# romi/plant-3d-vision

Hardware: AMD Instinct MI355X
Metric: Mvoxels*views/sec space-carve, 512^3 x 72 views per MI355X (higher is better)
Workload: dtype f32

## Files before the change

### include/spacecarve_tuning.h

```cpp
#ifndef SPACECARVE_TUNING_H
#define SPACECARVE_TUNING_H

#define SC_OPT_COMPACT 5

#define SC_OPT_DENSE_VIEWS 6
#define SC_OPT_STAGE1_VIEWS 7
#define SC_OPT_LIST_BLOCKS 8
#define SC_OPT_VIEW_GROUP 9
#define SC_OPT_BRICK 10
#define SC_OPT_STAGE2_VIEWS 12
#define SC_OPT_PACK_ROWS 13
#define SC_OPT_DEFER_STORES 14
#define SC_OPT_DEFER_SHARE 15
#define SC_OPT_FULL_BRICKS 19
#define SC_OPT_AVG_BRICK 20
#define SC_OPT_AVG_TILE_F32 29
#define SC_OPT_STAGE1_STORE_SHARE 17
#define SC_OPT_STAGE1_LIST_BLOCKS 21
#define SC_OPT_PACK_RIDE 22
#define SC_OPT_BRICK_WALKERS 23
#define SC_OPT_FILL_BLOCKS 25
#define SC_OPT_FINAL_VOXELS 24
#define SC_OPT_VIEW_BRICK 26
#define SC_OPT_STAGE1_VOXELS 30
#define SC_OPT_FLAG_VIEWS 11
#define SC_OPT_BULK_MIN 32
#define SC_OPT_ITEM_BIAS 33
#define SC_OPT_UNIT_BLOCKS 34
#define SC_OPT_BULK_FLOOR 35
#define SC_OPT_BULK_ADAPT SC_OPT_BULK_FLOOR

#define SC_OPT_LIST_CAP 38
#define SC_OPT_HOST_PACK 39
#define SC_OPT_HOST_THREADS 40
#define SC_OPT_LDS_TILES 41
#define SC_OPT_BULK_LIVE 42
#define SC_OPT_SAFE_KERNELS 43
#define SC_OPT_DENSE_EXTRA 44
#define SC_OPT_SPEC_SHARE 45
#define SC_OPT_SPEC_BLOCKS 46
#define SC_OPT_LATE_ROAD 47
#define SC_OPT_UNIT_CULL 37

#endif
```

### plant-3d-vision_amd/_native.py

```python
import ctypes
import importlib.util
import os
import subprocess
import sys
import threading

import numpy as np

_PKG_DIR = os.path.dirname(os.path.abspath(__file__))
LIB_PATH = os.path.join(_PKG_DIR, "libspacecarve.so")
_ALT_LIB = os.environ.get("SPACECARVE_LIB", "")
if _ALT_LIB:
    LIB_PATH = os.path.abspath(_ALT_LIB)
HEADER_PATH = os.path.join(os.path.dirname(_PKG_DIR), "include", "spacecarve.h")

SC_OK = 0
SC_ERR_INVALID, SC_ERR_DEVICE, SC_ERR_NOMEM, SC_ERR_STATE = -1, -2, -3, -4
SC_MODE_CARVE, SC_MODE_AVERAGE = 0, 1
SC_CREATE_DEFERRED = 1
SC_MASK_U8, SC_MASK_I32, SC_MASK_F32, SC_MASK_U8_INV, SC_MASK_BOOL_INV = 0, 1, 2, 3, 4
SC_MASK_U8_LUT = 5
SC_OPT_VIEWS_PER_LAUNCH, SC_OPT_VIEW_ORDER, SC_OPT_TIME_KERNELS, SC_OPT_MAX_PENDING = 1, 2, 3, 4
SC_OPT_COMPACT, SC_OPT_DENSE_VIEWS, SC_OPT_STAGE1_VIEWS, SC_OPT_LIST_BLOCKS = 5, 6, 7, 8
SC_OPT_VIEW_GROUP, SC_OPT_BRICK, SC_OPT_FLAG_VIEWS, SC_OPT_STAGE2_VIEWS = 9, 10, 11, 12
SC_KERNEL_CARVE, SC_KERNEL_AVERAGE, SC_KERNEL_PACK, SC_KERNEL_FILL, SC_KERNEL_LIST = 0, 1, 2, 3, 4
SC_KERNEL_FLAGS, SC_KERNEL_STEP = 5, 6
SC_OPT_PACK_ROWS, SC_OPT_DEFER_STORES, SC_OPT_DEFER_SHARE = 13, 14, 15
SC_OPT_FULL_BRICKS, SC_OPT_AVG_BRICK = 19, 20
SC_OPT_STAGE1_STORE_SHARE, SC_OPT_STAGE1_LIST_BLOCKS = 17, 21
SC_OPT_PACK_RIDE, SC_OPT_BRICK_WALKERS, SC_OPT_FILL_BLOCKS, SC_OPT_FINAL_VOXELS = 22, 23, 25, 24
SC_OPT_VIEW_BRICK, SC_OPT_AVG_TILE_F32, SC_OPT_STAGE1_VOXELS, SC_OPT_RESERVE_EVENTS = 26, 29, 30, 31
SC_OPT_BULK_MIN, SC_OPT_ITEM_BIAS, SC_OPT_UNIT_BLOCKS, SC_OPT_BULK_FLOOR = 32, 33, 34, 35
SC_OPT_BULK_ADAPT = SC_OPT_BULK_FLOOR
SC_OPT_UNIT_CULL, SC_OPT_LIST_CAP, SC_OPT_HOST_PACK, SC_OPT_HOST_THREADS, SC_OPT_LDS_TILES, SC_OPT_BULK_LIVE, SC_OPT_SAFE_KERNELS = 37, 38, 39, 40, 41, 42, 43
SC_OPT_DENSE_EXTRA = 44
SC_OPT_SPEC_SHARE, SC_OPT_SPEC_BLOCKS, SC_OPT_LATE_ROAD = 45, 46, 47
SC_FILTER_LINEAR, SC_FILTER_EXCESS_GREEN = 0, 1
SC_FOOT = {"t0": 0, "t90": 1, "t180": 2, "t270": 3, "diamond": 4, "square": 5}

_SIGNATURES = {
    "sc_abi_version": ("i", []),
    "sc_last_error": ("s", []),
    "sc_device_count": ("i", ["p"]),
    "sc_create": ("i", ["p", "q", "q", "q", "p", "f", "i", "f", "i"]),
    "sc_create_slab": ("i", ["p", "q", "q", "q", "q", "q", "p", "f", "i", "f", "i"]),
    "sc_create_cyclic": ("i", ["p", "q", "q", "q", "q", "q", "p", "f", "i", "f", "i"]),
    "sc_prewarm": ("i", ["i"]),
    "sc_prewarm_wait": ("v", []),
    "sc_create_ex": ("i", ["p", "q", "q", "q", "q", "q", "q", "p", "f", "i", "f", "i", "i"]),
    "sc_setup_times": ("i", ["p", "p"]),
    "sc_destroy": ("v", ["p"]),
    "sc_clear": ("i", ["p"]),
    "sc_set_option": ("i", ["p", "i", "q"]),
    "sc_set_stream": ("i", ["p", "p"]),
    "sc_order_after": ("i", ["p", "p"]),
    "sc_order_before": ("i", ["p", "p"]),
    "sc_set_lut": ("i", ["p", "p"]),
    "sc_process_view": ("i", ["p", "p", "p", "p", "p", "i", "i", "i", "q"]),
    "sc_process_views": ("i", ["p", "i", "p", "p", "p", "p", "i", "i", "i", "q"]),
    "sc_process_views_device": ("i", ["p", "i", "p", "p", "p", "p", "i", "i", "i"]),
    "sc_process_png_views": ("i", ["p", "i", "p", "p", "p", "p", "p", "i", "i"]),
    "sc_average_labels": ("i", ["p", "i", "i", "p", "p", "p", "p", "i", "i"]),
    "sc_average_labels_fused_count": ("q", []),
    "sc_flush": ("i", ["p"]),
    "sc_synchronize": ("i", ["p"]),
    "sc_get_values": ("i", ["p", "p"]),
    "sc_get_values_i8": ("i", ["p", "p"]),
    "sc_values_device_ptr": ("i", ["p", "p"]),
    "sc_num_voxels": ("q", ["p"]),
# ... 988 lines not shown
```

### plant-3d-vision_amd/csrc/sc_bricks.h

```cpp

template <bool ALL_SAFE = false>
__device__ __forceinline__ void two_views(const ViewDesc &da, const ViewDesc &db, bool two, float x, float y,
                                          const float (&z)[4], unsigned long long (&alive)[4], unsigned long long (&kept)[4]) {
    const float aax = da.R[0] * x + da.R[1] * y, aay = da.R[3] * x + da.R[4] * y, aaz = da.R[6] * x + da.R[7] * y;
    const float bax = db.R[0] * x + db.R[1] * y, bay = db.R[3] * x + db.R[4] * y, baz = db.R[6] * x + db.R[7] * y;
    const uint32_t rowa = (uint32_t)da.strip, rowb = (uint32_t)db.strip;
    unsigned long long oka[4], okb[4];
    uint32_t wa[4], wb[4];
    int sha[4], shb[4];
#pragma unroll
    for (int e = 0; e < 4; ++e) {
        int v;
        bool ok = project<ALL_SAFE>(aax, aay, aaz, z[e], da, sha[e], v, oka[e]);
        wa[e] = load_mask_at(da.mask, ok ? mask_byte_offset(sha[e], v, rowa) : 0u);
        ok = project<ALL_SAFE>(bax, bay, baz, z[e], db, shb[e], v, okb[e]);
        wb[e] = load_mask_at(db.mask, ok ? mask_byte_offset(shb[e], v, rowb) : 0u);
    }
    const unsigned long long second = two ? ~0ull : 0ull;
#pragma unroll
    for (int e = 0; e < 4; ++e) {
        unsigned long long fg = __ballot(__builtin_amdgcn_ubfe(wa[e], (uint32_t)sha[e], 1u) != 0u);
        unsigned long long seen = oka[e] & alive[e];
        alive[e] &= ~(seen & ~fg);
        kept[e] |= seen & fg;
// ... 138 lines not shown
        unsigned long long body = culled & ~last;
        while (body != 0) {
            const uint32_t bz = (uint32_t)__builtin_ctzll(body);
            body &= body - 1;
            asm volatile("global_store_dwordx4 %0, %1, %2 nt" ::"v"(voff), "v"(minus), "s"(wbase + bz * 256u) : "memory");
        }
        if ((culled & last) != 0 && tail_ok)
            asm volatile("global_store_dwordx4 %0, %1, %2 nt" ::"v"(voff), "v"(minus), "s"(wbase + (bricks_z - 1u) * 256u) : "memory");
        asm volatile("s_nop 1" ::"v"(minus));
    }
    unsigned long long rest = full | untouched;
    if (rest == 0) return;
    int32_t *col = labels + ((uint64_t)il * g.ny + j) * g.nzp;
    while (rest != 0) {
        const uint32_t bz = (uint32_t)__builtin_ctzll(rest);
        rest &= rest - 1;
        const bool isfull = (full >> bz) & 1ull;
        const uint32_t k0 = bz * kBrickZ + l16 * 4;
        if (k0 >= g.nz) continue;
        if (!isfull || fill.fresh) {
            const int32_t val = isfull ? fill.kept : fill.init;
            const v4i vv = {val, val, val, val};
            __builtin_nontemporal_store(vv, reinterpret_cast<v4i *>(col + k0));
        } else {
            const uint32_t n = min(4u, g.nz - k0);
            for (uint32_t e = 0; e < n; ++e)
                if (col[k0 + e] == 0) col[k0 + e] = 1;
        }
    }
}

#ifdef SC_TRACE_DENSE
__device__ uint32_t g_dense_trace[8192 * 8];
#endif
constexpr int kConfirmWaves = 8;
struct UnitRoad {
    int32_t *labels;
    int32_t init, fresh;
    uint32_t nbricks;
};

__global__ __launch_bounds__(64 * kConfirmWaves) void brick_confirm_kernel(
    GridDesc g, const ViewDesc *__restrict__ views, int v0, int v1, uint32_t bricks_y, uint32_t bricks_z,
    uint8_t *__restrict__ flags, const uint32_t *__restrict__ cands, uint32_t cand_per, uint32_t *__restrict__ late,
    ListCtl *ctl, uint32_t parity, UnitRoad ur) {
    if (v0 >= v1) return;
    uint32_t ncand[kCandSub], gfirst[kCandSub + 1];
    gfirst[0] = 0;
#pragma unroll
    for (int s = 0; s < kCandSub; ++s) {
        ncand[s] = ctl->ncand[parity][s].n;
        gfirst[s + 1] = gfirst[s] + ((ncand[s] + 63u) >> 6);
    }
    __shared__ unsigned long long s_full[kConfirmWaves], s_seen[kConfirmWaves];
    __shared__ unsigned long long s_road, s_rseen;
    const uint32_t wave = __builtin_amdgcn_readfirstlane(threadIdx.x >> 6), lane = threadIdx.x & 63u;
    const uint32_t per_plane = bricks_y * bricks_z;
    for (uint32_t grp = blockIdx.x; grp < gfirst[kCandSub]; grp += gridDim.x) {
        uint32_t sub = 0, first = 0, n = ncand[0];
#pragma unroll
        for (int s = 1; s < kCandSub; ++s)
            if (grp >= gfirst[s]) { sub = (uint32_t)s; first = gfirst[s]; n = ncand[s]; }
        const uint32_t idx = (grp - first) * 64u + lane;
        const bool isc = idx < n;
        const uint32_t lb = isc ? cands[(size_t)sub * cand_per * 64u + idx] : 0u;
        const uint32_t fl = isc ? flags[lb] : 0u;
// ... 43 lines not shown
                const uint32_t src = (uint32_t)__builtin_ctzll(mm);
                const uint32_t b = __builtin_amdgcn_readlane(lb, src);
                const bool seen = (ms >> src) & 1ull;
                const uint32_t bil = b / per_plane, brem = b - bil * per_plane;
                const uint32_t bby = brem / bricks_z, bbz = brem - bby * bricks_z;
                const uint32_t k0 = bbz * kBrickZ + (lane & 15u) * 4u;
#pragma unroll
                for (uint32_t i = 0; i < 4u; ++i) {
                    const uint32_t j = bby * kBrickY + i * 4u + (lane >> 4);
                    if (j >= g.ny || k0 >= g.nz) continue;
                    int32_t *p = ur.labels + ((uint64_t)bil * g.ny + j) * g.nzp + k0;
                    if (ur.fresh) {
                        const int32_t val = (seen && ur.init == 0) ? 1 : ur.init;
                        *reinterpret_cast<int4 *>(p) = make_int4(val, val, val, val);
                    } else if (seen) {
                        int4 q = *reinterpret_cast<const int4 *>(p);
                        const bool changed = q.x == 0 || q.y == 0 || q.z == 0 || q.w == 0;
                        q.x = q.x == 0 ? 1 : q.x; q.y = q.y == 0 ? 1 : q.y; q.z = q.z == 0 ? 1 : q.z; q.w = q.w == 0 ? 1 : q.w;
                        if (changed) *reinterpret_cast<int4 *>(p) = q;
                    }
                }
            }
        }
        __syncthreads();
    }
}

template <bool FRESH, bool ALL_SAFE = false>
__global__ __launch_bounds__(kBlock) __attribute__((amdgpu_num_sgpr(102))) void carve_brick_kernel(int32_t *__restrict__ labels, GridDesc g,
                                                             const ViewDesc *__restrict__ views,
                                                             int nviews, int32_t init, Append ap,
                                                             uint32_t bricks_y, uint32_t bricks_z,
                                                             const uint8_t *__restrict__ flags,
                                                             const uint32_t *__restrict__ live,
                                                             ListCtl *ctl, uint32_t nwalkers,
                                                             PackJob ride, int pack_rows,
                                                             uint32_t parity, int nverd_arg, uint32_t verd_max_live,
                                                             uint32_t bulk_min_live, int nextra) {
    if (blockIdx.x >= nwalkers) {
        const uint32_t b = blockIdx.x - nwalkers;
        if (pack_rows == 0) pack_band_block(ride, b);
        else if (pack_rows == 1) pack16_block<1>(ride, b);
        else if (pack_rows == 2) pack16_block<2>(ride, b);
        else if (pack_rows == 8) pack16_block<8>(ride, b);
        else pack16_block<4>(ride, b);
        return;
    }
    const uint32_t nlive = ctl->nlive[parity];
    const int nverd = nlive <= verd_max_live ? nverd_arg : 0;
    if (nlive < bulk_min_live) ap.bulk = nullptr;
    const uint32_t lane = threadIdx.x & 63;
    const uint32_t per_plane = bricks_y * bricks_z;
    const uint32_t xcd = blockIdx.x & 7u;
    const uint32_t per_xcd = (nwalkers >> 3) * (kBlock / 64);
    bool first = true;
    uint32_t misses = 0, turn = 0;
#ifdef SC_TRACE_DENSE
    const uint64_t tr0 = wall_clock64();
    uint32_t tr_bricks = 0, tr_units = 0, tr_verd = 0, tr_unit = 0, tr_tick = 0;
#endif
    for (;;) {
#ifdef SC_TRACE_DENSE
        const uint64_t tra = wall_clock64();
#endif
        uint32_t t = (blockIdx.x >> 3) * (kBlock / 64) + (threadIdx.x >> 6);
        if (!first) {
            const uint32_t nc = min(8u, per_xcd);
            const uint32_t c = t % nc;
            uint32_t n = 0;
            if (lane == 0) n = atomicAdd(&ctl->xcd_next[xcd * 8u + c].n, 1u);
            n = __builtin_amdgcn_readfirstlane(n);
            t = per_xcd + ((n / kXcdRun) * nc + c) * kXcdRun + (n % kXcdRun);
        }
        first = false;
        t = __builtin_amdgcn_readfirstlane(t);
        const uint32_t entry = ((t / kXcdRun) * 8u + xcd) * kXcdRun + (t % kXcdRun);
        if ((t / kXcdRun) * 8u * kXcdRun >= nlive) break;
        if (entry >= nlive) continue;
        const uint32_t lb = __builtin_amdgcn_readfirstlane(live[entry]);
        const uint32_t il = lb / per_plane;
        const uint32_t rem = lb - il * per_plane;
        const uint32_t by = rem / bricks_z, bz = rem - by * bricks_z;
        uint32_t culled = 0;
#ifdef SC_TRACE_DENSE
        const uint64_t trb = wall_clock64();
        tr_tick += (uint32_t)(trb - tra);
        ++tr_bricks;
#endif
        const bool ask = nverd > 0 && (misses < 8u || (turn & 7u) == 0u);
        ++turn;
        if (ask) {
            const uint32_t u = lane >> 4, vq = lane & 15u;
            uint32_t v = 0u;
            if ((int)vq < nverd) {
                const ViewDesc d = views[vq];
                const float x = g.ox + (float)(int)(il * g.istride + g.i0) * g.vs;
                v = rect_verdict_cells(d, g, x, (int)(by * kBrickY), (int)(by * kBrickY) + kBrickY - 1,
                                       (int)(bz * kBrickZ + u * 16u), (int)(bz * kBrickZ + u * 16u) + 15);
            }
            const unsigned long long e = __ballot(v == 1u);
            culled = ((e & 0xffffull) ? 1u : 0u) | (((e >> 16) & 0xffffull) ? 2u : 0u) |
                     (((e >> 32) & 0xffffull) ? 4u : 0u) | ((e >> 48) ? 8u : 0u);
            misses = culled ? 0u : misses + 1u;
        }
#ifdef SC_TRACE_DENSE
        const uint64_t trc = wall_clock64();
        tr_verd += (uint32_t)(trc - trb);
#endif
        const uint32_t j = by * kBrickY + (lane >> 2);
        for (uint32_t u = 0; u < 4u; ++u) {
            const uint32_t k0 = bz * kBrickZ + u * 16u + (lane & 3u) * 4u;
            if ((culled >> u) & 1u) {
                if (j < g.ny && k0 < g.nz)
                    *reinterpret_cast<int4 *>(labels + ((uint64_t)il * g.ny + j) * g.nzp + k0) = make_int4(-1, -1, -1, -1);
                continue;
            }
            brick_voxels<FRESH, ALL_SAFE>(labels, g, views, nviews, init, ap, il, j, k0, lb, lane, u, nextra);
#ifdef SC_TRACE_DENSE
            ++tr_units;
#endif
        }
#ifdef SC_TRACE_DENSE
        tr_unit += (uint32_t)(wall_clock64() - trc);
#endif
    }
#ifdef SC_TRACE_DENSE
    if (lane == 0) {
        const uint32_t w = blockIdx.x * 4u + (threadIdx.x >> 6);
        if (w < 8192u) {
            uint32_t *o = g_dense_trace + w * 8u;
            o[0] = (uint32_t)tr0; o[1] = (uint32_t)wall_clock64(); o[2] = tr_bricks; o[3] = tr_units;
            o[4] = tr_verd; o[5] = tr_unit; o[6] = tr_tick; o[7] = 0;
        }
    }
#endif
}

template <bool FRESH>
__global__ __launch_bounds__(kBlock) __attribute__((amdgpu_num_sgpr(102))) void carve_brick_light_kernel(
    int32_t *__restrict__ labels, GridDesc g, const ViewDesc *__restrict__ views, int nviews, int32_t init,
    uint32_t bricks_y, uint32_t bricks_z, const uint32_t *__restrict__ live, const uint32_t *__restrict__ fill_list,
    const ListCtl *ctl, uint32_t nwalkers, uint32_t parity) {
    const uint32_t wave = __builtin_amdgcn_readfirstlane(threadIdx.x >> 6), lane = threadIdx.x & 63;
    const uint32_t per_plane = bricks_y * bricks_z;
    if (blockIdx.x >= nwalkers) {
        const uint32_t nfill = ctl->nfill[parity], nfillers = gridDim.x - nwalkers;
        const bool vec = (g.nzp & 3u) == 0;
        const int32_t kept = init == 0 ? 1 : init;
        for (uint32_t base = (blockIdx.x - nwalkers) * 64u; base < nfill; base += nfillers * 64u) {
            const uint32_t mine = (base + lane < nfill) ? fill_list[base + lane] : 0u;
            const uint32_t n = min(64u, nfill - base);
            for (uint32_t q = 0; q < n; ++q) {
                const uint32_t ent = __builtin_amdgcn_readlane(mine, q);
                const bool isfull = (ent >> 31) != 0, isunt = ((ent >> 30) & 1u) != 0;
                if (isunt && !FRESH) continue;
                const uint32_t lb = ent & 0x3fffffffu;
                const uint32_t il = lb / per_plane;
                const uint32_t rem = lb - il * per_plane;
                const uint32_t by = rem / bricks_z, bz = rem - by * bricks_z;
                const uint32_t j = by * kBrickY + wave * 4 + (lane >> 4), k0 = bz * kBrickZ + (lane & 15) * 4;
                if (j >= g.ny || k0 >= g.nz) continue;
                int32_t *p = labels + ((uint64_t)il * g.ny + j) * g.nzp + k0;
                const uint32_t nv4 = min(4u, g.nz - k0);
                if (!isfull || FRESH) {
                    const int32_t val = isunt ? init : (isfull ? kept : -1);
                    if (vec) {
                        typedef int v4i __attribute__((ext_vector_type(4)));
                        v4i vv = {val, val, val, val};
                        __builtin_nontemporal_store(vv, reinterpret_cast<v4i *>(p));
                    } else {
                        for (uint32_t e = 0; e < nv4; ++e) p[e] = val;
                    }
                } else {
                    for (uint32_t e = 0; e < nv4; ++e)
                        if (p[e] == 0) p[e] = 1;
                }
            }
        }
        return;
    }
    const uint32_t nlive = ctl->nlive[parity];
    const Append none{nullptr, nullptr, 0u, 0u, nullptr, 0u, 0u};
    const uint32_t xcd = blockIdx.x & 7u, seq = blockIdx.x >> 3, per_xcd = nwalkers >> 3;
    for (uint32_t t = seq; ; t += per_xcd) {
        const uint32_t entry = ((t / kXcdRun) * 8u + xcd) * kXcdRun + (t % kXcdRun);
        if ((t / kXcdRun) * 8u * kXcdRun >= nlive) break;
        if (entry >= nlive) continue;
        const uint32_t lb = live[entry];
        const uint32_t il = lb / per_plane;
        const uint32_t rem = lb - il * per_plane;
        const uint32_t by = rem / bricks_z, bz = rem - by * bricks_z;
        const uint32_t j = by * kBrickY + wave * 4 + (lane >> 4);
        brick_voxels<FRESH>(labels, g, views, nviews, init, none, il, j, bz * kBrickZ + (lane & 15) * 4, lb, lane);
    }
}

template <bool FRESH, bool VEC>
__global__ __launch_bounds__(kBlock) void carve_kernel_1(int32_t *__restrict__ labels, GridDesc g,
                                                         ViewDesc view, int32_t init) {
    static_assert(VEC, "rows are whole 16-byte groups: the state is always read and written as int4");
    constexpr int G = !FRESH ? kStreamGroups : 1;
    uint32_t lb = spread_block(blockIdx.x, gridDim.x);
    uint64_t grp = (uint64_t)lb * (kBlock * G) + threadIdx.x;
    Append none{nullptr, nullptr, 0u, 0u, nullptr, 0u, 0u};
    int4 cur = make_int4(-1, -1, -1, -1);
    typedef int v4i __attribute__((ext_vector_type(4)));
    auto stream_load = [&](uint64_t gidx) {
        v4i q = __builtin_nontemporal_load(reinterpret_cast<const v4i *>(labels + gidx * 4));
        return make_int4(q.x, q.y, q.z, q.w);
    };
    if (!FRESH && grp < g.ngroups) cur = stream_load(grp);
#pragma unroll 1
    for (int s = 0; s < G; ++s, grp += kBlock) {
        int4 nxt = make_int4(-1, -1, -1, -1);
        if (G > 1 && s + 1 < G && grp + kBlock < g.ngroups)
            nxt = stream_load(grp + kBlock);
        if (grp < g.ngroups) carve_group<FRESH>(labels, g, &view, 1, init, grp, cur, none);
        cur = nxt;
    }
}
```

### plant-3d-vision_amd/csrc/sc_engine.h

```cpp

struct sc_engine {
    int device = 0;
    int mode = SC_MODE_CARVE;
    int64_t nx = 0, ny = 0, nz = 0, i0 = 0, istride = 1, planes = 0, n = 0;
    int64_t nzp = 0;
    int64_t npitch = 0;
    void *dense = nullptr;
    float origin[3] = {0, 0, 0};
    float vs = 1.0f;
    float default_value = 0.0f;
    void *state = nullptr;
    bool fresh = true;

    hipStream_t own_stream = nullptr, stream = nullptr;
    std::thread setup_thread;
    bool setup_pending = false;
    int setup_rc = SC_OK;
    std::string setup_err;
    double setup_ms = 0.0;
    double setup_waited_ms = 0.0;

    std::vector<ViewDesc> pending;
    ViewDesc *views_dev = nullptr;
    ViewDesc *views_pin = nullptr;
// ... 32 lines not shown
    bool sparse_late = false;
    hipEvent_t sparse_busy[2] = {nullptr, nullptr}, packed_busy = nullptr;
    bool sparse_busy_armed[2] = {false, false}, packed_busy_armed = false;
    size_t packed_cap = 0;
    SparseHeader *sparse_hdr_pin[2] = {nullptr, nullptr};
    size_t wire_stage_words = 0;
    int64_t unit_cull = 1;
    uint32_t *late = nullptr;
    uint32_t *bulk = nullptr;
    uint32_t bulkcap = 0;
    int64_t bulk_min = 128;
    bool last_bulk = false;
    uint4 *items = nullptr;
    uint32_t itemcap = 0;
    int64_t bulk_floor = 8192;
    int64_t bulk_live = 2;
    int64_t list_cap = 0, list_cap_built = 0;
    uint32_t *fill_list = nullptr;
    uint64_t flag_launches = 0;
    uint32_t last_parity = 0;
    struct DeferredBatch {
        bool on = false;
        const void *raw = nullptr;
        int V = 0, H = 0, W = 0, dtype = 0;
        int64_t row_stride = 0, view_stride = 0;
    } deferred;
    int64_t flag_views = 8;
    float *lut_dev = nullptr;

    uint32_t *lists = nullptr;
    ListCtl *ctl = nullptr;
    uint32_t subcap = 0;

    int64_t late_road = 1;
    int64_t safe_kernels = 1;
    int64_t host_pack = 1;
    struct HostBits {
        char *pin = nullptr, *dev = nullptr;
        size_t cap = 0, used = 0;
        hipEvent_t ev = nullptr;
        bool armed = false;
    } hb[2];
    int hb_cur = 0;
    std::vector<BitsRec> hp_pending;

    void *pin[kSlots] = {nullptr, nullptr, nullptr, nullptr};
    void *raw[kSlots] = {nullptr, nullptr, nullptr, nullptr};
    hipEvent_t slot_ev[kSlots] = {nullptr, nullptr, nullptr, nullptr};
    bool slot_armed[kSlots] = {false, false, false, false};
    size_t slot_bytes = 0;
    int next_slot = 0;

    int64_t views_per_launch = 0;
    int64_t view_order = 1;
    int64_t time_kernels = 0;
    int64_t max_pending = 256;
    int64_t compact = 1;
    int64_t brick = 1;
    int64_t dense_views = 2;
    int64_t stage1_views = 6;

    std::vector<TimedLaunch> timed[kNumKernels];
    hipEvent_t step_start = nullptr;
    bool step_open = false;
    hipEvent_t span_start = nullptr;
    bool span_open = false;
// ... 711 lines not shown
```

### plant-3d-vision_amd/csrc/sc_sparse.h

```cpp

constexpr uint32_t kSparseMagic = 0x50534353u;
constexpr uint32_t kSparseBrickBytes = kBrickY * kBrickZ / 4;
constexpr uint32_t kSparseMixed = 2u;

struct SparseHeader {
    uint32_t magic, version, bits, nbricks;
    uint32_t cap, nmixed, planes, ny;
    uint32_t nz, bricks_y, bricks_z, first;
    uint32_t stride;
    uint32_t nread;
    uint32_t pad[2];
};
static_assert(sizeof(SparseHeader) == 64, "SparseHeader layout");

struct SparseLayout {
    uint64_t codes, ids, payload, total;
};
__host__ __device__ inline SparseLayout sparse_layout(uint32_t nbricks, uint32_t cap) {
    SparseLayout l;
    l.codes = 64;
    l.ids = l.codes + (((uint64_t)nbricks + 63u) & ~(uint64_t)63u);
    l.payload = l.ids + (((uint64_t)cap * 4u + 63u) & ~(uint64_t)63u);
    l.total = l.payload + (uint64_t)cap * kSparseBrickBytes;
    return l;
}

struct SparseCounters {
    uint32_t nmixed, pad0[31];
    uint32_t nwork, pad1[31];
    uint32_t done, pad2[31];
};

struct SparseScan {
    const uint8_t *flags;
    uint32_t nbricks;
    int32_t level;
    uint32_t code_full, code_untouched;
    uint32_t *work;
};
struct SparseLists {
    const uint32_t *list0, *list1, *list2;
    const uint32_t *count0, *count1, *count2;
    int32_t step0, step1, step2;
};

constexpr uint32_t kSparseTurn = 8;

__global__ __launch_bounds__(kBlock) void sparse_pack_kernel(const int32_t *__restrict__ labels, GridDesc g, uint32_t bricks_y,
                                                            uint32_t bricks_z, SparseScan sc, uint32_t nscan, SparseLists sl,
                                                            char *__restrict__ wire, SparseHeader hdr, SparseCounters *cnt,
                                                            SparseCounters *cnt_next) {
    const SparseLayout lay = sparse_layout(hdr.nbricks, hdr.cap);
    uint8_t *codes = reinterpret_cast<uint8_t *>(wire + lay.codes);
    const uint32_t lane = threadIdx.x & 63u;
    const unsigned long long below = (lane == 0) ? 0ull : (~0ull >> (64 - lane));
    if (blockIdx.x < nscan) {
        const uint32_t b = blockIdx.x * kBlock + threadIdx.x;
        bool unknown = false;
        if (b < sc.nbricks) {
            uint32_t code = kSparseMixed;
            if (sc.level == 2) {
                const uint32_t f = sc.flags[b];
                code = (f == 1u || f == 4u) ? 3u : (f == 2u ? sc.code_full : (f == 6u ? sc.code_untouched : kSparseMixed));
            } else if (sc.level == 1) {
                code = sc.flags[b] != 0 ? 3u : kSparseMixed;
            }
            unknown = code == kSparseMixed;
            if (!unknown) codes[b] = (uint8_t)code;
        }
        if (sc.work != nullptr) {
            const unsigned long long m = __ballot(unknown);
            if (m != 0) {
                uint32_t base = 0;
                if (lane == 0) base = atomicAdd(&cnt->nwork, (uint32_t)__popcll(m));
                base = __shfl(base, 0);
                if (unknown) sc.work[base + (uint32_t)__popcll(m & below)] = b;
            }
        }
        return;
    }
    if (blockIdx.x == nscan && threadIdx.x == 0 && cnt_next != nullptr) {
        cnt_next->nmixed = 0u;
        cnt_next->nwork = 0u;
        cnt_next->done = 0u;
    }
    uint32_t *ids = reinterpret_cast<uint32_t *>(wire + lay.ids);
    uint32_t *payload = reinterpret_cast<uint32_t *>(wire + lay.payload);
    __shared__ uint32_t s_mixed[kBlock / 64], s_base;
    const uint32_t wave = __builtin_amdgcn_readfirstlane(threadIdx.x >> 6);
    const uint32_t npack = gridDim.x - nscan;
    uint32_t n0 = 0, n1 = 0, n2 = 0;
    if (sl.list0 != nullptr) n0 = *sl.count0;
    if (sl.list1 != nullptr) n1 = *sl.count1;
    if (sl.list2 != nullptr) n2 = *sl.count2;
    n0 = min(n0, hdr.nbricks); n1 = min(n1, hdr.nbricks); n2 = min(n2, hdr.nbricks);
    const uint32_t total = n0 + n1 + n2;
    const uint32_t per_plane = bricks_y * bricks_z;
    const uint32_t jl = lane >> 2, kq = (lane & 3u) * 16u;
    constexpr uint32_t kBlockTurn = kSparseTurn * (kBlock / 64);
    for (uint32_t tb = (blockIdx.x - nscan) * kBlockTurn; tb < total; tb += npack * kBlockTurn) {
        uint32_t mine = 0xffffffffu, j0 = 0, kb = 0, off_lo = 0, off_hi = 0;
        {
            const uint32_t t = tb + wave * kSparseTurn + lane;
            if (lane < kSparseTurn && t < total) {
                const uint32_t *lp = t < n0 ? sl.list0 : (t < n0 + n1 ? sl.list1 : sl.list2);
                const int64_t at = t < n0 ? (int64_t)t * sl.step0
                                          : (t < n0 + n1 ? (int64_t)(t - n0) * sl.step1 : (int64_t)(t - n0 - n1) * sl.step2);
                mine = lp[at];
                if (mine >= hdr.nbricks) mine = 0xffffffffu;
            }
            if (mine != 0xffffffffu) {
                const uint32_t il = mine / per_plane, rem = mine - il * per_plane;
                const uint32_t by = rem / bricks_z, bz = rem - by * bricks_z;
                j0 = by * kBrickY;
                kb = bz * kBrickZ;
                const uint64_t off = ((uint64_t)il * g.ny + j0) * g.nzp + kb;
                off_lo = (uint32_t)off;
                off_hi = (uint32_t)(off >> 32);
            }
        }
        uint32_t w[kSparseTurn];
        uint32_t codes2 = 0, mixed = 0;
        constexpr uint32_t kFlight = 8;
#pragma unroll
        for (uint32_t s8 = 0; s8 < kSparseTurn; s8 += kFlight) {
            int4 q[kFlight][4];
            uint32_t bj[kFlight], bk[kFlight];
            bool have[kFlight];
#pragma unroll
            for (uint32_t i = 0; i < kFlight; ++i) {
                have[i] = __builtin_amdgcn_readlane(mine, s8 + i) != 0xffffffffu;
                bj[i] = __builtin_amdgcn_readlane(j0, s8 + i);
                bk[i] = __builtin_amdgcn_readlane(kb, s8 + i);
                const uint64_t off = ((uint64_t)__builtin_amdgcn_readlane(off_hi, s8 + i) << 32) | __builtin_amdgcn_readlane(off_lo, s8 + i);
                const int32_t *p = labels + off + (uint64_t)jl * g.nzp + kq;
                const bool row_ok = have[i] && bj[i] + jl < g.ny;
#pragma unroll
                for (int e = 0; e < 4; ++e) {
                    const int32_t *pe = (row_ok && bk[i] + kq + 4u * e < g.nz) ? p + 4 * e : labels;
                    q[i][e] = *reinterpret_cast<const int4 *>(pe);
// ... 136 lines not shown
```

### plant-3d-vision_amd/csrc/sc_types.h

```cpp


struct ViewDesc {
    float K[4];
    float R[9];
    float t[3];
    const void *mask;
    int32_t W, H;
    int32_t tiles_x;
    int32_t pad;
    float Wf, Hf;
    const uint8_t *occ;
    int32_t safe;
    int32_t strip;
    const uint32_t *cmask;
    uint64_t reserved;
};
static_assert(sizeof(ViewDesc) == 128, "ViewDesc layout");
__device__ __forceinline__ ViewDesc scalar_desc(const ViewDesc *views, uint32_t i) {
#if defined(__HIP_DEVICE_COMPILE__)
    typedef const __attribute__((address_space(4))) ViewDesc *const_views_t;
    return ((const_views_t)(uintptr_t)views)[__builtin_amdgcn_readfirstlane(i)];
#else
    return views[i];
#endif
// ... 15 lines not shown
    FastDiv by_nzp, by_ny;
};

constexpr int kBlock = 256;
constexpr int kTile = 32;
constexpr int kSub = 256;
constexpr int kStreamGroups = 2;
constexpr int kXcdRun = 16;
constexpr int kCandSub = 8;

constexpr uint32_t kListBlocks = 2048;
constexpr uint32_t kBrickWalkers = 1280;
constexpr uint32_t kFinalListBlocks = 1536;
constexpr uint32_t kStoreBlocks = 256;
constexpr uint32_t kStage1StoreShare = 5;
constexpr uint32_t kStage1ListBlocks = 1280;
constexpr uint32_t kSpecShare = 3;
constexpr uint32_t kSpecBlocks = 64;
constexpr uint32_t kUnitBlocks = 512;
constexpr uint32_t kItemBias = 12;
constexpr int kViewGroup = 2;

struct alignas(128) ListCounter {
    uint32_t n;
    uint32_t cut;
    uint32_t pad[30];
};
__device__ __forceinline__ uint32_t list_count(const ListCounter &c, uint32_t cap) {
    return min(min(c.n, cap), c.cut ? ~c.cut : 0xffffffffu);
}
struct ListCtl {
    ListCounter count[5][kSub];
    uint32_t overflow;
    uint32_t nlive[2];
    uint32_t nlate;
    uint32_t nfill[2];
    uint32_t nlate_units;
    uint32_t pad[25];
    ListCounter xcd_next[64];
    ListCounter ncand[2][kCandSub];
};

struct CullStores {
    const uint8_t *flags;
    uint32_t bricks_y, bricks_z, nstrips, first;
    int32_t kept, fresh;
    uint32_t fill_blocks;
    int32_t init;
    uint32_t spec;
};
```

### plant-3d-vision_amd/csrc/sc_verdicts.h

```cpp

constexpr int kBrickY = 16, kBrickZ = 64;

struct PixelBox {
    float umin, umax, vmin, vmax;
    bool inside;
    bool outside;
};

__device__ __forceinline__ PixelBox rect_box(const ViewDesc &d, const GridDesc &g, float x, int j0, int j1, int k0, int k1) {
    PixelBox bx{0.0f, 0.0f, 0.0f, 0.0f, false, false};
    const float y0 = g.oy + (float)j0 * g.vs, y1 = g.oy + (float)j1 * g.vs;
    const float z0 = g.oz + (float)k0 * g.vs, z1 = g.oz + (float)k1 * g.vs;
    float p[3][4], e[3];
#pragma unroll
    for (int r = 0; r < 3; ++r) {
        const int q = r == 0 ? 6 : (r == 1 ? 0 : 3);
        const float tt = d.t[r == 0 ? 2 : (r == 1 ? 0 : 1)];
        const float a = d.R[q] * x, b0 = d.R[q + 1] * y0, b1 = d.R[q + 1] * y1, c0 = d.R[q + 2] * z0, c1 = d.R[q + 2] * z1;
        const float s0 = a + b0, s1 = a + b1;
        p[r][0] = (s0 + c0) + tt;
        p[r][1] = (s0 + c1) + tt;
        p[r][2] = (s1 + c0) + tt;
        p[r][3] = (s1 + c1) + tt;
        e[r] = (((fabsf(a) + fmaxf(fabsf(b0), fabsf(b1))) + fmaxf(fabsf(c0), fabsf(c1))) + fabsf(tt)) * 0x1p-19f;
// ... 131 lines not shown
            for (int tx = fpr.tx0; tx <= fpr.tx1; ++tx) {
                uint32_t o = load_occ(d.occ, (uint32_t)(ty * occ_tx + tx));
                any |= o;
                all &= o;
            }
    }
    return (any & 1u) == 0 ? 1u : ((all & 2u) != 0 ? 2u : 0u);
}

__device__ __forceinline__ uint32_t brick_flat_f32(const ViewDesc &d, const GridDesc &g, float x, int j0, int k0,
                                                   uint32_t &bits, bool *all_inside = nullptr) {
    const Footprint fpr = brick_footprint(d, g, x, j0, k0);
    if (all_inside != nullptr) *all_inside = fpr.inside;
    bits = 0u;
    if (fpr.outside) return 4u;
    if (!fpr.ok) return 0u;
    const int otx = (d.W + 31) >> 5, oty = (d.H + 31) >> 5;
    const uint32_t *val = reinterpret_cast<const uint32_t *>(d.occ + (((size_t)otx * oty + 3) & ~(size_t)3));
    const uint32_t first = load_cells(val, (uint32_t)(fpr.ty0 * otx + fpr.tx0));
    bool flat = true;
    for (int ty = fpr.ty0; ty <= fpr.ty1; ++ty)
        for (int tx = fpr.tx0; tx <= fpr.tx1; ++tx)
            flat &= load_occ(d.occ, (uint32_t)(ty * otx + tx)) != 0 && load_cells(val, (uint32_t)(ty * otx + tx)) == first;
    bits = first;
    return flat ? 3u : 0u;
}

constexpr int kFlagWaves = 8;

struct FlagViews { ViewDesc v[kFlagWaves]; };
struct DescCopy { const uint32_t *src; uint32_t *dst; uint32_t words; };
struct SpecFill { int32_t *labels; uint64_t bytes; uint32_t nblocks; };

__global__ __launch_bounds__(64 * kFlagWaves) void brick_flags_kernel(
    GridDesc g, const ViewDesc *__restrict__ views, int nviews, uint32_t bricks_y, uint32_t bricks_z,
    uint32_t nbricks, uint8_t *__restrict__ flags, uint32_t *__restrict__ live, ListCtl *ctl,
    FlagViews own, DescCopy dc, const ViewDesc *__restrict__ allviews, int nall, int nbatch,
    uint8_t *__restrict__ dead, int dead_stale, uint32_t parity, uint32_t *__restrict__ fill_list, SpecFill sf,
    uint32_t *__restrict__ cands, uint32_t cand_per) {
    __shared__ unsigned long long s_empty[kFlagWaves], s_full[kFlagWaves], s_seen[kFlagWaves];
    if (blockIdx.x < sf.nblocks) {
        typedef int v4i __attribute__((ext_vector_type(4)));
        const v4i minus = {-1, -1, -1, -1};
        char *base = reinterpret_cast<char *>(sf.labels);
        for (uint64_t off = ((uint64_t)blockIdx.x * (64 * kFlagWaves) + threadIdx.x) * 16u; off < sf.bytes;
             off += (uint64_t)sf.nblocks * (64 * kFlagWaves * 16))
            __builtin_nontemporal_store(minus, reinterpret_cast<v4i *>(base + off));
        return;
    }
    const uint32_t bid = blockIdx.x - sf.nblocks;
    if (bid == 0) {
        for (uint32_t i = threadIdx.x; i < dc.words; i += 64 * kFlagWaves) dc.dst[i] = dc.src[i];
        if (threadIdx.x == 0) ctl->nlive[parity ^ 1u] = ctl->nfill[parity ^ 1u] = 0u;
        if (threadIdx.x < (uint32_t)kCandSub) ctl->ncand[parity ^ 1u][threadIdx.x].n = 0u;
    }
    const uint32_t wave = __builtin_amdgcn_readfirstlane(threadIdx.x >> 6), lane = threadIdx.x & 63u;
    const uint32_t lb = bid * 64u + lane;
    const bool inb = lb < nbricks;
    const bool isdead = inb && dead != nullptr && !dead_stale && dead[lb] != 0;
    const bool valid = inb && !isdead;
    const uint32_t per_plane = bricks_y * bricks_z;
    const uint32_t il = lb / per_plane;
    const uint32_t rem = lb - il * per_plane;
    const uint32_t by = rem / bricks_z, bz = rem - by * bricks_z;
    const float x = g.ox + (float)(int)(il * g.istride + g.i0) * g.vs;
    const int j0 = (int)(by * kBrickY), k0 = (int)(bz * kBrickZ);
    bool empty = false, full = true, seen = false;
    if (valid) {
        if (views == nullptr) {
            if ((int)wave < nviews) {
                const uint32_t v = brick_verdict(own.v[wave], g, x, j0, k0, own.v[wave].tiles_x);
                empty = v == 1u;
                full = v == 2u || v == 4u;
                seen = v == 2u;
            }
        } else {
            for (int vi = (int)wave; vi < nviews; vi += kFlagWaves) {
                const ViewDesc d = views[vi];
                const uint32_t v = brick_verdict(d, g, x, j0, k0, d.tiles_x);
                empty |= v == 1u;
                full &= v == 2u || v == 4u;
                seen |= v == 2u;
            }
        }
    }
    unsigned long long any_empty = 0, cand = 0, any_seen = 0;
    {
        const unsigned long long me = __ballot(empty), mf = __ballot(full && valid), ms = __ballot(seen);
        if (lane == 0) { s_empty[wave] = me; s_full[wave] = mf; s_seen[wave] = ms; }
        __syncthreads();
        cand = ~0ull;
#pragma unroll
        for (int w = 0; w < kFlagWaves; ++w) { any_empty |= s_empty[w]; cand &= s_full[w]; any_seen |= s_seen[w]; }
        cand &= ~any_empty;
    }
    for (int base = nviews; base < nall && cand != 0; base += kFlagWaves) {
        const int vi = base + (int)wave;
        bool e2 = false, f2 = true, s2 = false;
        if (vi < nall && ((cand >> lane) & 1ull)) {
            const ViewDesc d = allviews[vi];
            const uint32_t v = brick_verdict(d, g, x, j0, k0, d.tiles_x);
            e2 = v == 1u;
            f2 = v == 2u || v == 4u;
            s2 = v == 2u;
        }
        const unsigned long long me = __ballot(e2), mf = __ballot(f2), ms = __ballot(s2);
        __syncthreads();
        if (lane == 0) { s_empty[wave] = me; s_full[wave] = mf; s_seen[wave] = ms; }
        __syncthreads();
#pragma unroll
        for (int w = 0; w < kFlagWaves; ++w) { any_empty |= s_empty[w]; cand &= s_full[w]; any_seen |= s_seen[w]; }
        cand &= ~any_empty;
    }
    if (nall <= 0) cand = 0;
    if (wave != 0) return;
    const bool gone = (any_empty >> lane) & 1ull, kept = (cand >> lane) & 1ull, saw = (any_seen >> lane) & 1ull;
    if (inb) flags[lb] = isdead ? 4 : (gone ? 1 : (kept ? (nall >= nbatch ? (saw ? 2 : 6) : (saw ? 3 : 7)) : 0));
    if (valid && dead != nullptr && (gone || dead_stale)) dead[lb] = gone ? 1 : 0;
    const bool alive = valid && !gone && !kept;
    const unsigned long long m = __ballot(alive);
    const unsigned long long below = (lane == 0) ? 0ull : (~0ull >> (64 - lane));
    if (m != 0) {
        uint32_t base = 0;
        if (lane == 0) base = atomicAdd(&ctl->nlive[parity], (uint32_t)__popcll(m));
        base = __shfl(base, 0);
        if (alive) live[base + (uint32_t)__popcll(m & below)] = lb;
    }
    const bool open = cands != nullptr && nall < nbatch && inb && !isdead && !gone && kept;
    const unsigned long long mc = __ballot(open);
    if (mc != 0) {
        const uint32_t sub = bid / cand_per;
        uint32_t base = 0;
        if (lane == 0) base = atomicAdd(&ctl->ncand[parity][sub].n, (uint32_t)__popcll(mc));
        base = __shfl(base, 0);
        if (open) cands[(size_t)sub * cand_per * 64u + base + (uint32_t)__popcll(mc & below)] = lb;
    }
    if (fill_list != nullptr) {
        const bool fillme = valid && (gone || kept);
        const unsigned long long mf = __ballot(fillme);
        if (mf != 0) {
            uint32_t base = 0;
            if (lane == 0) base = atomicAdd(&ctl->nfill[parity], (uint32_t)__popcll(mf));
            base = __shfl(base, 0);
            const unsigned long long below = (lane == 0) ? 0ull : (~0ull >> (64 - lane));
            if (fillme) fill_list[base + (uint32_t)__popcll(mf & below)] = lb | (gone ? 0u : (saw ? 0x80000000u : 0x40000000u));
        }
    }
}
```

### plant-3d-vision_amd/csrc/spacecarve.hip

```cpp

#include <hip/hip_runtime.h>

#include "hostwait.h"

#include <algorithm>
#include <atomic>
#include <chrono>
#include <cmath>
#include <condition_variable>
#include <cstdarg>
#include <cstdio>
#include <cstdlib>
#include <cstring>
#include <mutex>
#include <new>
#include <string>
#include <thread>
#include <vector>

#include "hostpack.h"
#include "spacecarve.h"
#include "spacecarve_tuning.h"

namespace sctrace {
// ... 55 lines not shown
        hipError_t _e = (expr);                                                              \
        if (_e != hipSuccess)                                                                \
            return fail(_e == hipErrorOutOfMemory ? SC_ERR_NOMEM : SC_ERR_DEVICE,            \
                        "%s failed: %s (%s:%d)", #expr, hipGetErrorString(_e), __FILE__,     \
                        __LINE__);                                                           \
    } while (0)

struct Chunk {
    char *base = nullptr;
    size_t cap = 0, used = 0;
};

struct TimedLaunch {
    hipEvent_t start, stop;
};

constexpr int kSlots = 4;
constexpr int kNumKernels = 7;

}

#include "sc_engine.h"
#include "sc_flush.inl"


#include "sc_api_engine.inl"
#include "sc_api_values.inl"
#include "sc_api_group.inl"

#ifdef SC_TRACE_DENSE
extern "C" int sc_debug_dense_trace(uint32_t *out) {
    return (int)hipMemcpyFromSymbol(out, HIP_SYMBOL(g_dense_trace), sizeof(uint32_t) * 8192 * 8);
}
#endif

#include "sc_api_sparse.inl"
#include "sc_comm.inl"
```

Baseline: 66.19 million.

## Split live brick list into heavy-front and light-back halves by neighbour count

The live-brick counter becomes a packed 64-bit pair, so the flags kernel can write bricks it classes as 'heavy' from the front of the list and the rest from the back. The carve walkers then visit the heavy bricks first. A new order option picks the heuristic: neighbour count, or a count of views in which the brick is fully inside the silhouette (trace builds only). The sparse pack path gains a fourth list slot, and trace buffers are added. With the default order of zero every brick counts as heavy, so the layout is as before, apart from a 64-bit atomic and extra index logic.

```diff
diff --git a/include/spacecarve_tuning.h b/include/spacecarve_tuning.h
--- a/include/spacecarve_tuning.h
+++ b/include/spacecarve_tuning.h
@@ -40,6 +40,7 @@
 #define SC_OPT_SPEC_SHARE 45
 #define SC_OPT_SPEC_BLOCKS 46
 #define SC_OPT_LATE_ROAD 47
+#define SC_OPT_LIVE_ORDER 48
 #define SC_OPT_UNIT_CULL 37
 
 #endif
diff --git a/plant-3d-vision_amd/_native.py b/plant-3d-vision_amd/_native.py
--- a/plant-3d-vision_amd/_native.py
+++ b/plant-3d-vision_amd/_native.py
@@ -35,6 +35,7 @@
 SC_OPT_UNIT_CULL, SC_OPT_LIST_CAP, SC_OPT_HOST_PACK, SC_OPT_HOST_THREADS, SC_OPT_LDS_TILES, SC_OPT_BULK_LIVE, SC_OPT_SAFE_KERNELS = 37, 38, 39, 40, 41, 42, 43
 SC_OPT_DENSE_EXTRA = 44
 SC_OPT_SPEC_SHARE, SC_OPT_SPEC_BLOCKS, SC_OPT_LATE_ROAD = 45, 46, 47
+SC_OPT_LIVE_ORDER = 48
 SC_FILTER_LINEAR, SC_FILTER_EXCESS_GREEN = 0, 1
 SC_FOOT = {"t0": 0, "t90": 1, "t180": 2, "t270": 3, "diamond": 4, "square": 5}
 
diff --git a/plant-3d-vision_amd/csrc/sc_bricks.h b/plant-3d-vision_amd/csrc/sc_bricks.h
--- a/plant-3d-vision_amd/csrc/sc_bricks.h
+++ b/plant-3d-vision_amd/csrc/sc_bricks.h
@@ -194,6 +194,7 @@
 
 #ifdef SC_TRACE_DENSE
 __device__ uint32_t g_dense_trace[8192 * 8];
+__device__ uint32_t g_brick_trace[32768 * 4];
 #endif
 constexpr int kConfirmWaves = 8;
 struct UnitRoad {
@@ -303,7 +304,7 @@
                                                              int nviews, int32_t init, Append ap,
                                                              uint32_t bricks_y, uint32_t bricks_z,
                                                              const uint8_t *__restrict__ flags,
-                                                             const uint32_t *__restrict__ live,
+                                                             const uint32_t *__restrict__ live, uint32_t live_room,
                                                              ListCtl *ctl, uint32_t nwalkers,
                                                              PackJob ride, int pack_rows,
                                                              uint32_t parity, int nverd_arg, uint32_t verd_max_live,
@@ -317,7 +318,9 @@
         else pack16_block<4>(ride, b);
         return;
     }
-    const uint32_t nlive = ctl->nlive[parity];
+    LiveList ll{live, live_room, 0u, 0u};
+    ll.count(ctl, parity);
+    const uint32_t nlive = ll.total;
     const int nverd = nlive <= verd_max_live ? nverd_arg : 0;
     if (nlive < bulk_min_live) ap.bulk = nullptr;
     const uint32_t lane = threadIdx.x & 63;
@@ -348,7 +351,7 @@
         const uint32_t entry = ((t / kXcdRun) * 8u + xcd) * kXcdRun + (t % kXcdRun);
         if ((t / kXcdRun) * 8u * kXcdRun >= nlive) break;
         if (entry >= nlive) continue;
-        const uint32_t lb = __builtin_amdgcn_readfirstlane(live[entry]);
+        const uint32_t lb = __builtin_amdgcn_readfirstlane(ll.at(entry));
         const uint32_t il = lb / per_plane;
         const uint32_t rem = lb - il * per_plane;
         const uint32_t by = rem / bricks_z, bz = rem - by * bricks_z;
@@ -392,7 +395,15 @@
 #endif
         }
 #ifdef SC_TRACE_DENSE
-        tr_unit += (uint32_t)(wall_clock64() - trc);
+        const uint64_t trd = wall_clock64();
+        tr_unit += (uint32_t)(trd - trc);
+        if (lane == 0 && entry < 32768u) {
+            uint32_t *o = g_brick_trace + entry * 4u;
+            o[0] = lb;
+            o[1] = (uint32_t)__popc(~culled & 15u) | (min(turn - 1u, 255u) << 4) | ((blockIdx.x * 4u + (threadIdx.x >> 6)) << 12);
+            o[2] = (uint32_t)tra;
+            o[3] = (uint32_t)trd;
+        }
 #endif
     }
 #ifdef SC_TRACE_DENSE
@@ -410,8 +421,8 @@
 template <bool FRESH>
 __global__ __launch_bounds__(kBlock) __attribute__((amdgpu_num_sgpr(102))) void carve_brick_light_kernel(
     int32_t *__restrict__ labels, GridDesc g, const ViewDesc *__restrict__ views, int nviews, int32_t init,
-    uint32_t bricks_y, uint32_t bricks_z, const uint32_t *__restrict__ live, const uint32_t *__restrict__ fill_list,
-    const ListCtl *ctl, uint32_t nwalkers, uint32_t parity) {
+    uint32_t bricks_y, uint32_t bricks_z, const uint32_t *__restrict__ live, uint32_t live_room,
+    const uint32_t *__restrict__ fill_list, const ListCtl *ctl, uint32_t nwalkers, uint32_t parity) {
     const uint32_t wave = __builtin_amdgcn_readfirstlane(threadIdx.x >> 6), lane = threadIdx.x & 63;
     const uint32_t per_plane = bricks_y * bricks_z;
     if (blockIdx.x >= nwalkers) {
@@ -450,14 +461,16 @@
         }
         return;
     }
-    const uint32_t nlive = ctl->nlive[parity];
+    LiveList ll{live, live_room, 0u, 0u};
+    ll.count(ctl, parity);
+    const uint32_t nlive = ll.total;
     const Append none{nullptr, nullptr, 0u, 0u, nullptr, 0u, 0u};
     const uint32_t xcd = blockIdx.x & 7u, seq = blockIdx.x >> 3, per_xcd = nwalkers >> 3;
     for (uint32_t t = seq; ; t += per_xcd) {
         const uint32_t entry = ((t / kXcdRun) * 8u + xcd) * kXcdRun + (t % kXcdRun);
         if ((t / kXcdRun) * 8u * kXcdRun >= nlive) break;
         if (entry >= nlive) continue;
-        const uint32_t lb = live[entry];
+        const uint32_t lb = ll.at(entry);
         const uint32_t il = lb / per_plane;
         const uint32_t rem = lb - il * per_plane;
         const uint32_t by = rem / bricks_z, bz = rem - by * bricks_z;
diff --git a/plant-3d-vision_amd/csrc/sc_engine.h b/plant-3d-vision_amd/csrc/sc_engine.h
--- a/plant-3d-vision_amd/csrc/sc_engine.h
+++ b/plant-3d-vision_amd/csrc/sc_engine.h
@@ -88,6 +88,7 @@
     ListCtl *ctl = nullptr;
     uint32_t subcap = 0;
 
+    int64_t live_order = 0;
     int64_t late_road = 1;
     int64_t safe_kernels = 1;
     int64_t host_pack = 1;
diff --git a/plant-3d-vision_amd/csrc/sc_sparse.h b/plant-3d-vision_amd/csrc/sc_sparse.h
--- a/plant-3d-vision_amd/csrc/sc_sparse.h
+++ b/plant-3d-vision_amd/csrc/sc_sparse.h
@@ -39,9 +39,9 @@
     uint32_t *work;
 };
 struct SparseLists {
-    const uint32_t *list0, *list1, *list2;
-    const uint32_t *count0, *count1, *count2;
-    int32_t step0, step1, step2;
+    const uint32_t *list0, *list1, *list2, *list3;
+    const uint32_t *count0, *count1, *count2, *count3;
+    int32_t step0, step1, step2, step3;
 };
 
 constexpr uint32_t kSparseTurn = 8;
@@ -89,12 +89,14 @@
     __shared__ uint32_t s_mixed[kBlock / 64], s_base;
     const uint32_t wave = __builtin_amdgcn_readfirstlane(threadIdx.x >> 6);
     const uint32_t npack = gridDim.x - nscan;
-    uint32_t n0 = 0, n1 = 0, n2 = 0;
+    uint32_t n0 = 0, n1 = 0, n2 = 0, n3 = 0;
     if (sl.list0 != nullptr) n0 = *sl.count0;
     if (sl.list1 != nullptr) n1 = *sl.count1;
     if (sl.list2 != nullptr) n2 = *sl.count2;
+    if (sl.list3 != nullptr) n3 = *sl.count3;
     n0 = min(n0, hdr.nbricks); n1 = min(n1, hdr.nbricks); n2 = min(n2, hdr.nbricks);
-    const uint32_t total = n0 + n1 + n2;
+    n3 = min(n3, hdr.nbricks);
+    const uint32_t total = n0 + n1 + n2 + n3;
     const uint32_t per_plane = bricks_y * bricks_z;
     const uint32_t jl = lane >> 2, kq = (lane & 3u) * 16u;
     constexpr uint32_t kBlockTurn = kSparseTurn * (kBlock / 64);
@@ -103,9 +105,11 @@
         {
             const uint32_t t = tb + wave * kSparseTurn + lane;
             if (lane < kSparseTurn && t < total) {
-                const uint32_t *lp = t < n0 ? sl.list0 : (t < n0 + n1 ? sl.list1 : sl.list2);
+                const uint32_t n01 = n0 + n1, n012 = n01 + n2;
+                const uint32_t *lp = t < n0 ? sl.list0 : (t < n01 ? sl.list1 : (t < n012 ? sl.list2 : sl.list3));
                 const int64_t at = t < n0 ? (int64_t)t * sl.step0
-                                          : (t < n0 + n1 ? (int64_t)(t - n0) * sl.step1 : (int64_t)(t - n0 - n1) * sl.step2);
+                                          : (t < n01 ? (int64_t)(t - n0) * sl.step1
+                                                     : (t < n012 ? (int64_t)(t - n01) * sl.step2 : (int64_t)(t - n012) * sl.step3));
                 mine = lp[at];
                 if (mine >= hdr.nbricks) mine = 0xffffffffu;
             }
diff --git a/plant-3d-vision_amd/csrc/sc_types.h b/plant-3d-vision_amd/csrc/sc_types.h
--- a/plant-3d-vision_amd/csrc/sc_types.h
+++ b/plant-3d-vision_amd/csrc/sc_types.h
@@ -71,13 +71,26 @@
 struct ListCtl {
     ListCounter count[5][kSub];
     uint32_t overflow;
-    uint32_t nlive[2];
     uint32_t nlate;
     uint32_t nfill[2];
     uint32_t nlate_units;
-    uint32_t pad[25];
+    uint32_t pad0;
+    unsigned long long nlive[2];
+    uint32_t pad[22];
     ListCounter xcd_next[64];
     ListCounter ncand[2][kCandSub];
+};
+
+struct LiveList {
+    const uint32_t *list;
+    uint32_t room;
+    uint32_t heavy, total;
+    __device__ __forceinline__ void count(const ListCtl *ctl, uint32_t parity) {
+        const unsigned long long n = ctl->nlive[parity];
+        heavy = (uint32_t)n;
+        total = heavy + (uint32_t)(n >> 32);
+    }
+    __device__ __forceinline__ uint32_t at(uint32_t i) const { return list[i < heavy ? i : room - 1u - (i - heavy)]; }
 };
 
 struct CullStores {
diff --git a/plant-3d-vision_amd/csrc/sc_verdicts.h b/plant-3d-vision_amd/csrc/sc_verdicts.h
--- a/plant-3d-vision_amd/csrc/sc_verdicts.h
+++ b/plant-3d-vision_amd/csrc/sc_verdicts.h
@@ -187,12 +187,16 @@
 struct DescCopy { const uint32_t *src; uint32_t *dst; uint32_t words; };
 struct SpecFill { int32_t *labels; uint64_t bytes; uint32_t nblocks; };
 
+#ifdef SC_TRACE_DENSE
+__device__ uint32_t g_brick_proxy[1u << 20];
+#endif
+
 __global__ __launch_bounds__(64 * kFlagWaves) void brick_flags_kernel(
     GridDesc g, const ViewDesc *__restrict__ views, int nviews, uint32_t bricks_y, uint32_t bricks_z,
     uint32_t nbricks, uint8_t *__restrict__ flags, uint32_t *__restrict__ live, ListCtl *ctl,
     FlagViews own, DescCopy dc, const ViewDesc *__restrict__ allviews, int nall, int nbatch,
     uint8_t *__restrict__ dead, int dead_stale, uint32_t parity, uint32_t *__restrict__ fill_list, SpecFill sf,
-    uint32_t *__restrict__ cands, uint32_t cand_per) {
+    uint32_t *__restrict__ cands, uint32_t cand_per, uint32_t order) {
     __shared__ unsigned long long s_empty[kFlagWaves], s_full[kFlagWaves], s_seen[kFlagWaves];
     if (blockIdx.x < sf.nblocks) {
         typedef int v4i __attribute__((ext_vector_type(4)));
@@ -206,7 +210,10 @@
     const uint32_t bid = blockIdx.x - sf.nblocks;
     if (bid == 0) {
         for (uint32_t i = threadIdx.x; i < dc.words; i += 64 * kFlagWaves) dc.dst[i] = dc.src[i];
-        if (threadIdx.x == 0) ctl->nlive[parity ^ 1u] = ctl->nfill[parity ^ 1u] = 0u;
+        if (threadIdx.x == 0) {
+            ctl->nlive[parity ^ 1u] = 0ull;
+            ctl->nfill[parity ^ 1u] = 0u;
+        }
         if (threadIdx.x < (uint32_t)kCandSub) ctl->ncand[parity ^ 1u][threadIdx.x].n = 0u;
     }
     const uint32_t wave = __builtin_amdgcn_readfirstlane(threadIdx.x >> 6), lane = threadIdx.x & 63u;
@@ -249,6 +256,11 @@
         for (int w = 0; w < kFlagWaves; ++w) { any_empty |= s_empty[w]; cand &= s_full[w]; any_seen |= s_seen[w]; }
         cand &= ~any_empty;
     }
+#ifdef SC_TRACE_DENSE
+    uint32_t tr_nfull = 0;
+    if (wave == 0)
+        for (int w = 0; w < min(nviews, kFlagWaves); ++w) tr_nfull += (uint32_t)((s_full[w] >> lane) & 1ull);
+#endif
     for (int base = nviews; base < nall && cand != 0; base += kFlagWaves) {
         const int vi = base + (int)wave;
         bool e2 = false, f2 = true, s2 = false;
@@ -276,10 +288,27 @@
     const unsigned long long m = __ballot(alive);
     const unsigned long long below = (lane == 0) ? 0ull : (~0ull >> (64 - lane));
     if (m != 0) {
-        uint32_t base = 0;
-        if (lane == 0) base = atomicAdd(&ctl->nlive[parity], (uint32_t)__popcll(m));
-        base = __shfl(base, 0);
-        if (alive) live[base + (uint32_t)__popcll(m & below)] = lb;
+        uint32_t near = 0, unknown = 0;
+        {
+            const bool zl = bz > 0 && lane > 0, zr = bz + 1u < bricks_z && lane < 63u;
+            const bool yl = by > 0 && lane >= bricks_z, yr = by + 1u < bricks_y && lane + bricks_z < 64u;
+            near = (zl ? (uint32_t)((m >> (lane - 1u)) & 1ull) : 0u) + (zr ? (uint32_t)((m >> (lane + 1u)) & 1ull) : 0u) +
+                   (yl ? (uint32_t)((m >> (lane - bricks_z)) & 1ull) : 0u) + (yr ? (uint32_t)((m >> (lane + bricks_z)) & 1ull) : 0u);
+            unknown = 4u - ((zl ? 1u : 0u) + (zr ? 1u : 0u) + (yl ? 1u : 0u) + (yr ? 1u : 0u));
+        }
+        bool heavy = true;
+        const uint32_t kind = order >> 8, thr = order & 255u;
+        if (kind == 2u) heavy = near + unknown >= thr;
+        if (kind == 3u) heavy = near >= thr;
+#ifdef SC_TRACE_DENSE
+        if (kind == 1u) heavy = tr_nfull >= thr;
+        if (alive && lb < (1u << 20)) g_brick_proxy[lb] = tr_nfull | (near << 8) | (unknown << 16) | 0x80000000u;
+#endif
+        const unsigned long long mh = __ballot(alive && heavy), ml = m & ~mh;
+        unsigned long long base = 0;
+        if (lane == 0) base = atomicAdd(&ctl->nlive[parity], (unsigned long long)__popcll(mh) | ((unsigned long long)__popcll(ml) << 32));
+        const uint32_t bh = __builtin_amdgcn_readfirstlane((uint32_t)base), bl = __builtin_amdgcn_readfirstlane((uint32_t)(base >> 32));
+        if (alive) live[heavy ? bh + (uint32_t)__popcll(mh & below) : nbricks - 1u - (bl + (uint32_t)__popcll(ml & below))] = lb;
     }
     const bool open = cands != nullptr && nall < nbatch && inb && !isdead && !gone && kept;
     const unsigned long long mc = __ballot(open);
diff --git a/plant-3d-vision_amd/csrc/spacecarve.hip b/plant-3d-vision_amd/csrc/spacecarve.hip
--- a/plant-3d-vision_amd/csrc/spacecarve.hip
+++ b/plant-3d-vision_amd/csrc/spacecarve.hip
@@ -111,6 +111,11 @@
 extern "C" int sc_debug_dense_trace(uint32_t *out) {
     return (int)hipMemcpyFromSymbol(out, HIP_SYMBOL(g_dense_trace), sizeof(uint32_t) * 8192 * 8);
 }
+extern "C" int sc_debug_brick_trace(uint32_t *entries, uint32_t *proxy) {
+    int rc = (int)hipMemcpyFromSymbol(entries, HIP_SYMBOL(g_brick_trace), sizeof(uint32_t) * 32768 * 4);
+    if (rc == 0) rc = (int)hipMemcpyFromSymbol(proxy, HIP_SYMBOL(g_brick_proxy), sizeof(uint32_t) << 20);
+    return rc;
+}
 #endif
 
 #include "sc_api_sparse.inl"
```

After: 65.42 million. 0.988x the previous value.
